# chanchanchan97/ICAFusion

Hardware: AMD Instinct MI355X
Metric: RGB/IR image-pairs/sec (two-stream forward + NMS) (higher is better)
Workload: dtype bf16

## Files before the change

icafusion_amd/_lib.py:

```python
import ctypes as C
import os

_HERE = os.path.dirname(os.path.abspath(__file__))
LIB_PATH = os.environ.get("ICAF_LIB") or os.path.join(_HERE, "lib", "libicaf.so")

F32, BF16, F16 = 0, 1, 2
ACT_NONE, ACT_SILU, ACT_GELU = 0, 1, 2


class ConvArgs(C.Structure):
    _fields_ = [
        ("x", C.c_void_p), ("w", C.c_void_p), ("bias", C.c_void_p), ("y", C.c_void_p), ("res", C.c_void_p),
        ("x_gs", C.c_longlong), ("w_gs", C.c_longlong), ("bias_gs", C.c_longlong), ("y_gs", C.c_longlong),
        ("res_gs", C.c_longlong),
        ("groups", C.c_int),
        ("B", C.c_int), ("H", C.c_int), ("W", C.c_int), ("Cin", C.c_int), ("ldx", C.c_int),
        ("Ho", C.c_int), ("Wo", C.c_int), ("Cout", C.c_int), ("ldy", C.c_int),
        ("kh", C.c_int), ("kw", C.c_int), ("sh", C.c_int), ("sw", C.c_int), ("ph", C.c_int), ("pw", C.c_int),
        ("ldr", C.c_int), ("Kp", C.c_int), ("act", C.c_int), ("dtype", C.c_int), ("out_dtype", C.c_int),
        ("alpha_acc", C.c_float * 2), ("alpha_res", C.c_float * 2),
        ("tile", C.c_int),
        ("pre", C.c_void_p), ("pre_h", C.c_int), ("pre_w", C.c_int), ("ldpre", C.c_int), ("pre_mode", C.c_int),
        ("w2", C.c_void_p), ("bias2", C.c_void_p), ("y2", C.c_void_p),
        ("w2_gs", C.c_longlong), ("bias2_gs", C.c_longlong), ("y2_gs", C.c_longlong),
# ... 2 lines not shown
        ("x2", C.c_void_p), ("x2_gs", C.c_longlong), ("ldx2", C.c_int), ("reserved2", C.c_int),
    ]


class BneckArgs(C.Structure):
    _fields_ = [("conv", ConvArgs), ("w1", C.c_void_p), ("bias1", C.c_void_p), ("w1_gs", C.c_longlong),
                ("bias1_gs", C.c_longlong), ("Kp1", C.c_int), ("shape", C.c_int),
                ("x2", C.c_void_p), ("x2_gs", C.c_longlong), ("ldx2", C.c_int), ("reserved", C.c_int)]


class Stem2Args(C.Structure):
    _fields_ = [("img", C.c_void_p), ("img_u8", C.c_int), ("ctot", C.c_int),
                ("dtype", C.c_int), ("nstreams", C.c_int), ("B", C.c_int), ("H", C.c_int), ("W", C.c_int),
                ("w0", C.c_void_p), ("bias0", C.c_void_p), ("w0_gs", C.c_longlong), ("bias0_gs", C.c_longlong),
                ("Kp0", C.c_int), ("C0", C.c_int),
                ("w1", C.c_void_p), ("bias1", C.c_void_p), ("w1_gs", C.c_longlong), ("bias1_gs", C.c_longlong),
                ("Kp1", C.c_int), ("C1", C.c_int),
                ("w2", C.c_void_p), ("bias2", C.c_void_p), ("w2_gs", C.c_longlong), ("bias2_gs", C.c_longlong),
                ("Kp2", C.c_int), ("C2", C.c_int),
                ("y", C.c_void_p), ("y_gs", C.c_longlong), ("ldy", C.c_int), ("reserved", C.c_int)]


class DmffArgs(C.Structure):
    _fields_ = [("x", C.c_void_p), ("qkv", C.c_void_p), ("y", C.c_void_p),
                ("wqkv", C.c_void_p), ("bqkv", C.c_void_p), ("wo", C.c_void_p), ("bo", C.c_void_p),
                ("w1", C.c_void_p), ("b1", C.c_void_p), ("w2", C.c_void_p), ("b2", C.c_void_p),
                ("ln_attn_gamma", C.c_void_p * 2), ("ln_attn_beta", C.c_void_p * 2),
                ("ln_mlp_gamma", C.c_void_p), ("ln_mlp_beta", C.c_void_p),
                ("wqkv_gs", C.c_longlong), ("bqkv_gs", C.c_longlong), ("wo_gs", C.c_longlong), ("bo_gs", C.c_longlong),
                ("w1_gs", C.c_longlong), ("b1_gs", C.c_longlong), ("w2_gs", C.c_longlong), ("b2_gs", C.c_longlong),
                ("x_gs", C.c_longlong), ("y_gs", C.c_longlong),
                ("dtype", C.c_int), ("B", C.c_int), ("N", C.c_int), ("C", C.c_int), ("heads", C.c_int), ("Kp", C.c_int),
                ("Kp4", C.c_int), ("hidden", C.c_int), ("ldy", C.c_int), ("reserved", C.c_int),
                ("eps_attn", C.c_float), ("eps_mlp", C.c_float),
                ("coef_res_attn", C.c_float * 2), ("coef_acc_attn", C.c_float * 2),
                ("coef_res_mlp", C.c_float * 2), ("coef_acc_mlp", C.c_float * 2), ("debug_clock", C.c_void_p),
                ("x32", C.c_void_p), ("y32", C.c_void_p)]


_p, _i, _ll, _f, _sz = C.c_void_p, C.c_int, C.c_longlong, C.c_float, C.c_size_t
SIGNATURES = {
    "icaf_last_error": (C.c_char_p, []),
    "icaf_set_option": (_i, [C.c_char_p, _i]),
    "icaf_version": (_i, []),
    "icaf_device_info": (_i, [C.POINTER(_i), C.POINTER(_i), C.c_char_p, _i]),
    "icaf_preprocess_nchw": (_i, [_p, _p, _i, _i, _i, _i, _i, _i, _i, _p]),
    "icaf_preprocess_u8": (_i, [_p, _p, _i, _i, _i, _i, _i, _i, _i, _i, _i, _i, _p]),
    "icaf_stem": (_i, [_p, _i, _i, _p, _p, _p, _i, _i, _i, _i, _i, _i, _i, _i, _ll, _ll, _ll, _p]),
    "icaf_stem2": (_i, [C.POINTER(Stem2Args), _p]),
    "icaf_conv2d": (_i, [C.POINTER(ConvArgs), _p]),
    "icaf_bottleneck": (_i, [C.POINTER(BneckArgs), _p]),
    "icaf_conv2d_kernel_name": (_i, [C.POINTER(ConvArgs), C.c_char_p, _i]),
    "icaf_conv2d_config_ids": (_i, [C.POINTER(_i), _i]),
    "icaf_sppf_pool": (_i, [_p, _i, _p, _p, _p, _i, _i, _i, _i, _i, _i, _i, _p]),
    "icaf_sppf_config": (_i, [_i, _i, _i, _i, C.POINTER(_i)]),
    "icaf_upsample_nearest": (_i, [_p, _i, _p, _i, _i, _i, _i, _i, _i, _i, _p]),
    "icaf_copy_channels": (_i, [_p, _i, _p, _i, _i, _ll, _i, _p]),
    "icaf_axpby": (_i, [_p, _i, _p, _i, _p, _i, _i, _ll, _i, _f, _f, _p]),
    "icaf_dmff_pool_tokens": (_i, [_p, _i, _p, _i, _p, _p, _p, _i, _i, _i, _i, _i, _i, _i, _i, _i, _i, _i,
                                   _f, _f, _f, _f, _p]),
    "icaf_layernorm": (_i, [_p, _p, _p, _p, _p, _p, _i, _ll, _i, _i, _f, _p]),
    "icaf_cross_attention": (_i, [_p, _p, _i, _i, _i, _i, _i, _p]),
    "icaf_cross_attention_config": (_i, [_i, _i, _i, _i, _i, C.POINTER(_i), C.POINTER(_i), C.POINTER(_i)]),
    "icaf_dmff_ln_qkv": (_i, [C.POINTER(DmffArgs), _p]),
    "icaf_dmff_attn_mlp": (_i, [C.POINTER(DmffArgs), _p]),
    "icaf_dmff_wide_ln_qkv": (_i, [C.POINTER(DmffArgs), _p]),
    "icaf_dmff_wide_proj_mlp": (_i, [C.POINTER(DmffArgs), _p, _p]),
    "icaf_dmff_wide_proj_mlp_split": (_i, [C.POINTER(DmffArgs), _p, _p, _i, _p]),
    "icaf_dmff_wide_reduce": (_i, [C.POINTER(DmffArgs), _p, _i, _p]),
    "icaf_dmff_attn_mlp_lds_bytes": (_i, [_i, _i, _i, _i, C.POINTER(_sz)]),
    "icaf_dmff_upsample_merge": (_i, [_p, _p, _i, _p, _i, _p, _i, _i, _i, _i, _i, _i, _i, _i, _p]),
    "icaf_detect_decode": (_i, [_p, _i, _p, _p, _p, _i, _i, _i, _i, _i, _ll, _ll, _f, C.POINTER(_f), _p]),
    "icaf_detect_decode_kernel": (_i, [_p, _i, _p, _p, _i, _i, _i, _i, _i, C.POINTER(_i)]),
    "icaf_detect_conv": (_i, [C.POINTER(ConvArgs), _p, _p, _p, _i, _i, _ll, _ll, _f, C.POINTER(_f), _p]),
    "icaf_match_predictions": (_i, [_p, _p, _i, _i, _p, _p, _i, _p, _p, _i, _p, _p, _p]),
    "icaf_nms_workspace_bytes": (_i, [_i, _ll, _i, _i, C.POINTER(_sz)]),
    "icaf_nms": (_i, [_p, _i, _ll, _i, _f, _f, _i, _i, C.POINTER(_i), _i, _i, _i, _f, _p, _p, _p, _p, _sz, _p]),
    "icaf_graph_begin": (_i, [_p]),
    "icaf_graph_end": (_i, [_p, C.POINTER(_p)]),
    "icaf_graph_launch": (_i, [_p, _p]),
    "icaf_graph_destroy": (_i, [_p]),
    "icaf_event_create": (_i, [C.POINTER(_p)]),
    "icaf_event_record": (_i, [_p, _p]),
    "icaf_stream_wait_event": (_i, [_p, _p]),
    "icaf_event_elapsed_ms": (_i, [_p, _p, C.POINTER(_f)]),
    "icaf_event_destroy": (_i, [_p]),
    "icaf_stream_sync": (_i, [_p]),
}

_LIB = None


class IcafError(RuntimeError):
    pass


def lib():
    global _LIB
    if _LIB is None:
        if not os.path.exists(LIB_PATH):
            raise IcafError(f"{LIB_PATH} not found — build it with `python -m icafusion_amd.build` "
                            "(hipcc --offload-arch=gfx950); icafusion_amd has no CPU / PyTorch fallback")
        import torch
        handle = C.CDLL(LIB_PATH)
        for name, (res, args) in SIGNATURES.items():
            try:
# ... 17 lines not shown
```

icafusion_amd/csrc/conv_common.h:

```cpp
#pragma once
#include "icaf_common.h"

namespace icaf {

struct ConvP {
    const void* x; const void* w; const float* bias; void* y; const void* res;
    long long x_gs, w_gs, bias_gs, y_gs, res_gs;
    int B, H, W, Cin, ldx, Ho, Wo, Cout, ldy, kh, kw, sh, sw, ph, pw, ldr, Kp, act;
    int M, K, nchunks, mtiles, ntiles;
    int vec_y, vec_r;
    unsigned int x_bytes, w_bytes;
    float alpha_acc[2], alpha_res[2];
    const float* pre; int pre_h, pre_w, ldpre, pre_mode;
    const void* w1; const float* bias1;
    long long w1_gs, bias1_gs; int Kp1; unsigned int w1_bytes;
    const void* w2; const float* bias2; void* y2;
    long long w2_gs, bias2_gs, y2_gs; int Kp2, Cout2, ldy2, vec_y2, keep1; unsigned int w2_bytes;
    const void* x2; long long x2_gs; int ldx2;
};

constexpr int ROWB = 64;
constexpr int ROWS = 80;
constexpr int NTHREADS = 256;

int ctile_conv_check(const icaf_conv_args* a, const ConvP& p, int shape);
int launch_ctile(const icaf_conv_args* a, const ConvP& p, int shape, hipStream_t s);
const char* ctile_tag(int shape);
int stream_check(const icaf_conv_args* a, const ConvP& p, int shape);
int launch_stream(const icaf_conv_args* a, const ConvP& p, int shape, hipStream_t s);
const char* stream_tag(int shape);
int wreg_check(const icaf_conv_args* a, const ConvP& p, int shape);
int launch_wreg(const icaf_conv_args* a, const ConvP& p, int shape, hipStream_t s);
const char* wreg_tag(int shape);
int cstream_check(const icaf_conv_args* a, const ConvP& p, int shape);
int launch_cstream(const icaf_conv_args* a, const ConvP& p, int shape, hipStream_t s);
const char* cstream_tag(int shape);
int cwide_check(const icaf_conv_args* a, const ConvP& p, int shape);
int launch_cwide(const icaf_conv_args* a, const ConvP& p, int shape, hipStream_t s);
const char* cwide_tag(int shape);
int launch_bneck(const icaf_conv_args* a, const ConvP& p, int shape, hipStream_t s);

template <int ACT, int DT = ICAF_F32> __device__ __forceinline__ float apply_act(float v) {
    if constexpr (ACT == ICAF_ACT_SILU) return silu_f(v);
    else if constexpr (ACT == ICAF_ACT_GELU) return DT == ICAF_F32 ? gelu_f(v) : gelu_fast_f(v);
    else return v;
}
template <int ACT, int DT = ICAF_F32> __device__ __forceinline__ void apply_act4(const float (&x)[4], float (&y)[4]) {
    if constexpr (ACT == ICAF_ACT_SILU) silu4_f(x, y);
    else {
#pragma unroll
        for (int j = 0; j < 4; ++j) y[j] = apply_act<ACT, DT>(x[j]);
    }
}

__device__ __forceinline__ int xcd_tile(int ntile_total) {
    const int bid = blockIdx.x, q = ntile_total >> 3, r = ntile_total & 7, xcd = bid & 7, idx = bid >> 3;
    return (xcd < r ? xcd * (q + 1) : r * (q + 1) + (xcd - r) * q) + idx;
}

#ifndef ICAF_EPI_FAST
#define ICAF_EPI_FAST 1
#endif
// ... 400 lines not shown
```

icafusion_amd/csrc/detect.hip:

```cpp
#pragma clang fp contract(off)
#include "icaf_common.h"
#include "stream_core.h"
#include <cstdlib>

namespace icaf {

struct Anchors { float v[16]; };
int conv_prepare(const icaf_conv_args* a, ConvP& p);

struct DetectDiv { FastDiv no, nx, ny, na; };

template <bool I32>
__global__ __launch_bounds__(256) void detect_decode_kernel(const float* __restrict__ p, int ldp, float* __restrict__ z,
                                                            float* __restrict__ logits, float* __restrict__ raw, int B, int ny, int nx,
                                                            int na, int no, long long rows_total, long long row_offset, float stride,
                                                            Anchors anc, DetectDiv dv) {
    const long long total = (long long)B * na * ny * nx * no;
    for (long long e = (long long)blockIdx.x * blockDim.x + threadIdx.x; e < total; e += (long long)gridDim.x * blockDim.x) {
        int o, x, y, a, b;
        if constexpr (I32) {
            unsigned int q, r;
            fd_divmod((unsigned int)e, dv.no, q, r);
            o = (int)r;
            fd_divmod(q, dv.nx, q, r);
// ... 107 lines not shown
            const int nl = col0 + 8 * qd + 4 * hi;
#pragma unroll
            for (int b = 0; b < TM; ++b) {
                const int ml = row0 + b * 32 + l31;
                f32x4 v;
#pragma unroll
                for (int j = 0; j < 4; ++j) v[j] = acc[b][4 * qd + j] + bq[qd][j];
                *(f32x4*)(stg + ml * SO + nl * 4) = v;
            }
        }
    }
    __device__ __forceinline__ void flush(const unsigned char* stg, int m0, int n0, int tid) const {
        if (tid >= 128 * NA) return;
        const int row = tid / NA, a = tid - row * NA;
        const unsigned int pix = (unsigned int)(m0 + row);
        if ((int)pix >= M) return;
        unsigned int t, x, b, y;
        fd_divmod(pix, dnx, t, x);
        fd_divmod(t, dny, b, y);
        const float* src = (const float*)(stg + row * SO) + a * NO;
        float v[NO];
#pragma unroll
        for (int k = 0; k < NO; k += 2) { const float2 q2 = *(const float2*)(src + k); v[k] = q2.x; v[k + 1] = q2.y; }
        const long long cell = ((long long)a * ny + y) * nx + x;
        const long long zrow = (long long)b * rows_total + row_offset + cell;
        float o[NO];
#pragma unroll
        for (int k = 0; k < NO; ++k) {
            const float sg = 1.0f / (1.0f + expf(-v[k]));
            float out = sg;
            if (k == 0) out = ((sg * 2.0f - 0.5f) + (float)x) * stride;
            else if (k == 1) out = ((sg * 2.0f - 0.5f) + (float)y) * stride;
            else if (k == 2 || k == 3) {
                const float d = sg * 2.0f;
                out = (d * d) * anc.v[2 * a + (k - 2)];
            }
            o[k] = out;
        }
        float* zr = z + zrow * NO;
#pragma unroll
        for (int k = 0; k < NO; k += 2) *(float2*)(zr + k) = float2{o[k], o[k + 1]};
        if (raw) {
            float* rr = raw + (((long long)b * NA) * ny * nx + cell) * NO;
#pragma unroll
            for (int k = 0; k < NO; k += 2) *(float2*)(rr + k) = float2{v[k], v[k + 1]};
        }
        if (logits) {
#pragma unroll
            for (int k = 5; k < NO; ++k) logits[zrow * (NO - 5) + (k - 5)] = v[k];
        }
    }
};

template <int DT, int NA, int NO>
__global__ __launch_bounds__(512) void detect_conv_kernel(const ConvP p, const DetectEpi<NA, NO> epi) {
    stream_gemm<DT, 64, 1>(p, epi);
}

template <int DT, int NA, int NO>
static int launch_detect_conv(const ConvP& p, const DetectEpi<NA, NO>& epi, hipStream_t s) {
    constexpr int LDS = 3 * (128 + 64) * 128 + 128 * DetectEpi<NA, NO>::SO;
    ConvP q = p;
    q.mtiles = (p.M + 127) / 128;
    q.ntiles = 1;
    q.nchunks = p.K / 64;
    int dev = 0, cus = 256;
    ICAF_HIP(hipGetDevice(&dev));
    ICAF_HIP(hipDeviceGetAttribute(&cus, hipDeviceAttributeMultiprocessorCount, dev));
    const int grid = cus & ~7;
    ICAF_LDS_OPTIN((detect_conv_kernel<DT, NA, NO>), LDS);
    detect_conv_kernel<DT, NA, NO><<<dim3((unsigned)grid, 1, 1), dim3(512), LDS, s>>>(q, epi);
    ICAF_LAUNCH_CHECK();
    return ICAF_OK;
}

}

using namespace icaf;

enum { DETECT_PIXEL = 0, DETECT_ELEMENT = 1 };

static int detect_select(const float* p, int ldp, const float* z, const float* raw, int B, int ny, int nx, int na, int no) {
    const bool aligned = ldp % 2 == 0 && ((uintptr_t)p & 7) == 0 && ((uintptr_t)z & 7) == 0 && (!raw || ((uintptr_t)raw & 7) == 0);
    const bool pixel = na == 3 && (no == 6 || no == 8 || no == 14) && aligned && (long long)B * ny * nx < (1ll << 31) && !g_opt.detect_elementwise;
    return pixel ? DETECT_PIXEL : DETECT_ELEMENT;
}

extern "C" int icaf_detect_decode_kernel(const float* p, int ldp, const float* z, const float* raw, int B, int ny, int nx, int na, int no,
                                         int* kernel) {
    if (!p || !z || !kernel) return fail(ICAF_ERR_ARG, "icaf_detect_decode_kernel: null pointer");
    if (na < 1 || na > 8 || no < 6 || ldp < na * no) return fail(ICAF_ERR_ARG, "icaf_detect_decode_kernel: bad na/no/ldp");
    if (B < 1 || ny < 1 || nx < 1) return fail(ICAF_ERR_ARG, "icaf_detect_decode_kernel: empty level");
    *kernel = detect_select(p, ldp, z, raw, B, ny, nx, na, no);
    return ICAF_OK;
}

extern "C" int icaf_detect_decode(const float* p, int ldp, float* z, float* logits, float* raw, int B, int ny, int nx, int na, int no,
                                  long long rows_total, long long row_offset, float stride, const float* anchors_px, icaf_stream_t s) {
    if (!p || !z || !anchors_px) return fail(ICAF_ERR_ARG, "icaf_detect_decode: null pointer");
    if (na < 1 || na > 8 || no < 6 || ldp < na * no) return fail(ICAF_ERR_ARG, "icaf_detect_decode: bad na/no/ldp");
    if (row_offset + (long long)na * ny * nx > rows_total) return fail(ICAF_ERR_ARG, "icaf_detect_decode: level does not fit in z");
    Anchors anc;
    for (int i = 0; i < 16; ++i) anc.v[i] = i < 2 * na ? anchors_px[i] : 0.0f;
    const long long cells = (long long)B * na * ny * nx * no;
    long long blocks = (cells + 255) / 256;
    if (blocks > 256 * 32) blocks = 256 * 32;
    if (B < 1 || ny < 1 || nx < 1) return fail(ICAF_ERR_ARG, "icaf_detect_decode: empty level");
    if (detect_select(p, ldp, z, raw, B, ny, nx, na, no) == DETECT_PIXEL) {
        if (no == 6) return launch_detect_pixel<3, 6>(p, ldp, z, logits, raw, B, ny, nx, rows_total, row_offset, stride, anc, S(s));
        if (no == 8) return launch_detect_pixel<3, 8>(p, ldp, z, logits, raw, B, ny, nx, rows_total, row_offset, stride, anc, S(s));
        if (no == 14) return launch_detect_pixel<3, 14>(p, ldp, z, logits, raw, B, ny, nx, rows_total, row_offset, stride, anc, S(s));
    }
    const DetectDiv dv{make_fastdiv((unsigned)no), make_fastdiv((unsigned)nx), make_fastdiv((unsigned)ny), make_fastdiv((unsigned)na)};
    if (cells < (1ll << 31))
        hipLaunchKernelGGL(detect_decode_kernel<true>, dim3((unsigned)blocks), dim3(256), 0, S(s), p, ldp, z, logits, raw, B, ny, nx, na,
                           no, rows_total, row_offset, stride, anc, dv);
    else
        hipLaunchKernelGGL(detect_decode_kernel<false>, dim3((unsigned)blocks), dim3(256), 0, S(s), p, ldp, z, logits, raw, B, ny, nx, na,
                           no, rows_total, row_offset, stride, anc, dv);
    ICAF_LAUNCH_CHECK();
    return ICAF_OK;
}

extern "C" int icaf_detect_conv(const icaf_conv_args* a, float* z, float* logits, float* raw, int na, int no, long long rows_total,
// ... 27 lines not shown
```

icafusion_amd/csrc/igemm_stream.hip:

```cpp
#include "stream_core.h"

namespace icaf {

template <int DT, int BN, int ACT, bool PRE = false>
struct StoreEpi {
    using E = Elem<DT>;
    static constexpr int SO = BN * E::BYTES + 16;
    typename E::type* yg; float alpha_acc; int M, Cout, ldy;
    const typename E::type* rg; float alpha_res; int ldr;
    const float* pre; int pre_h, pre_w, ldpre, pre_mode, Ho, Wo;
    template <int TM>
    __device__ __forceinline__ void stage(const f32x16 (&acc)[TM], const f32x4 (&bq)[4], unsigned char* stg, int row0, int col0, int l31, int hi, int m0, int n0) const {
        const float* pt[PRE ? TM : 1][4];
        float plx[PRE ? TM : 1], ply[PRE ? TM : 1];
        if constexpr (PRE) {
#pragma clang fp contract(off)
            const float sy = (float)pre_h / (float)Ho, sx = (float)pre_w / (float)Wo;
#pragma unroll
            for (int b = 0; b < TM; ++b) {
                const int m = m0 + row0 + b * 32 + l31;
                const int mm = m < M ? m : 0;
                const int wo = mm % Wo, t = mm / Wo, ho = t % Ho, bi = t / Ho;
                float fy = ((float)ho + 0.5f) * sy - 0.5f, fx = ((float)wo + 0.5f) * sx - 0.5f;
                fy = fy < 0.0f ? 0.0f : fy;
// ... 24 lines not shown
                const int ml = row0 + b * 32 + l31;
                float pv[4] = {0.f, 0.f, 0.f, 0.f};
                if constexpr (PRE) if (n0 + nl < Cout) {
                    const f32x4 t00 = *(const f32x4*)(pt[b][0] + n0 + nl), t01 = *(const f32x4*)(pt[b][1] + n0 + nl);
                    const f32x4 t10 = *(const f32x4*)(pt[b][2] + n0 + nl), t11 = *(const f32x4*)(pt[b][3] + n0 + nl);
                    {
#pragma clang fp contract(off)
                        const float wx0 = 1.0f - plx[b], wy0 = 1.0f - ply[b];
#pragma unroll
                        for (int j = 0; j < 4; ++j) {
                            const float top = t00[j] * wx0 + t01[j] * plx[b];
                            const float bot = t10[j] * wx0 + t11[j] * plx[b];
                            pv[j] = top * wy0 + bot * ply[b];
                        }
                    }
                }
                float v[4];
#pragma unroll
                for (int j = 0; j < 4; ++j) v[j] = acc[b][4 * qd + j] + bq[qd][j] + pv[j];
                apply_act4<ACT, DT>(v, v);
#pragma unroll
                for (int j = 0; j < 4; ++j) v[j] *= alpha_acc;
                u32x2 pk;
                if constexpr (DT == ICAF_BF16) { pk[0] = pack2_bf16(v[0], v[1]); pk[1] = pack2_bf16(v[2], v[3]); }
                else { pk[0] = pack2_f16(v[0], v[1]); pk[1] = pack2_f16(v[2], v[3]); }
                *(u32x2*)(stg + ml * SO + nl * E::BYTES) = pk;
            }
        }
    }
    __device__ __forceinline__ void flush(const unsigned char* stg, int m0, int n0, int tid) const {
        constexpr int VPR = BN / E::VEC;
        constexpr int NIT = 128 * VPR / 512;
#pragma unroll
        for (int itv = 0; itv < NIT; ++itv) {
            const int idx = tid + itv * 512;
            const int row = idx / VPR, cv = idx - row * VPR;
            const int m = m0 + row, n = n0 + cv * E::VEC;
            u32x4 sv = *(const u32x4*)(stg + row * SO + cv * 16);
            if (m < M && n < Cout) {
                if (rg) {
                    float v[E::VEC], r[E::VEC];
                    unpack16<DT>(sv, v);
                    unpack16<DT>(*(const u32x4*)(rg + (long long)m * ldr + n), r);
#pragma unroll
                    for (int j = 0; j < E::VEC; ++j) v[j] = __builtin_fmaf(alpha_res, r[j], v[j]);
                    sv = pack16<DT>(v);
                }
                *(u32x4*)(yg + (long long)m * ldy + n) = sv;
            }
        }
    }
};

template <int DT, int BN, int ACT, int MODE, bool PRE = false>
__global__ __launch_bounds__(512) void igemm_stream_kernel(const ConvP p) {
    using E = Elem<DT>;
    const int g = blockIdx.z;
    const StoreEpi<DT, BN, ACT, PRE> epi{(typename E::type*)p.y + g * p.y_gs, p.alpha_acc[g], p.M, p.Cout, p.ldy,
                                         p.res ? (const typename E::type*)p.res + g * p.res_gs : nullptr, p.alpha_res[g], p.ldr,
                                         p.pre, p.pre_h, p.pre_w, p.ldpre, p.pre_mode, p.Ho, p.Wo};
    stream_gemm<DT, BN, MODE>(p, epi);
}

const char* stream_tag(int shape) { return shape == 1 ? "128x128" : shape == 2 ? "128x64" : "?"; }

static int stream_grid(int groups, int* wgx) {
    int dev = 0, cus = 256;
    ICAF_HIP(hipGetDevice(&dev));
    ICAF_HIP(hipDeviceGetAttribute(&cus, hipDeviceAttributeMultiprocessorCount, dev));
    *wgx = ((cus / (groups > 0 ? groups : 1)) & ~7) >> 3;
    return ICAF_OK;
}

int stream_check(const icaf_conv_args* a, const ConvP& p, int shape) {
    if (shape < 1 || shape > 2) return fail(ICAF_ERR_ARG, "igemm_stream: unknown shape %d", shape);
    if (a->dtype == ICAF_F32 || a->out_dtype != a->dtype) return fail(ICAF_ERR_UNSUPPORTED, "igemm_stream: 16-bit types, out dtype == dtype");
    if ((a->Cin * 2) % 128) return fail(ICAF_ERR_UNSUPPORTED, "igemm_stream: Cin * 2 bytes must be a multiple of 128 (Cin = %d)", a->Cin);
    if (a->w2) return fail(ICAF_ERR_UNSUPPORTED, "igemm_stream: no chained layer");
    if (a->pre && (a->act != ICAF_ACT_SILU || a->kh != 1 || a->kw != 1 || a->sh != 1 || a->sw != 1 || a->ph || a->pw || a->groups != 1))
        return fail(ICAF_ERR_UNSUPPORTED, "igemm_stream: the pre-activation term is built for 1x1 SiLU layers (one group)");
    if (a->res && !p.vec_r) return fail(ICAF_ERR_UNSUPPORTED, "igemm_stream: the residual must take 16-byte vectors");
    if (p.x_bytes == 0) return fail(ICAF_ERR_UNSUPPORTED, "igemm_stream: operand exceeds the 2 GiB buffer-descriptor range");
    if (!p.vec_y || a->Cout % 8) return fail(ICAF_ERR_UNSUPPORTED, "igemm_stream: y must take 16-byte vectors (ldy %% 8, Cout %% 8, alignment)");
    if (shape == 1 && a->Cout <= 64) return fail(ICAF_ERR_UNSUPPORTED, "igemm_stream 128x128: Cout = %d <= 64 (use 128x64)", a->Cout);
    int wgx = 0;
    const int st = stream_grid(a->groups, &wgx);
    if (st) return st;
    const int ntiles = (p.Cout + (shape == 1 ? 128 : 64) - 1) / (shape == 1 ? 128 : 64);
    if (wgx < ntiles || wgx % ntiles) return fail(ICAF_ERR_UNSUPPORTED, "igemm_stream: %d channel tiles do not divide the %d workgroups of an XCD", ntiles, wgx);
    return ICAF_OK;
}

template <int DT, int BN, int ACT>
static int launch_stream_cfg(const ConvP& p, int groups, hipStream_t s) {
    constexpr int LDS = 3 * (128 + BN) * 128 + 128 * (BN * 2 + 16);
    ConvP q = p;
    q.mtiles = (p.M + 127) / 128;
    q.ntiles = (p.Cout + BN - 1) / BN;
    q.nchunks = p.K / 64;
    int dev = 0, wgx = 0;
    ICAF_HIP(hipGetDevice(&dev));
    if (dev < 0 || dev >= ICAF_MAX_DEVICES) return fail(ICAF_ERR_UNSUPPORTED, "device ordinal %d", dev);
    int st = stream_grid(groups, &wgx);
    if (st) return st;
    const int grid = wgx << 3;
    if (wgx < q.ntiles || wgx % q.ntiles) return fail(ICAF_ERR_UNSUPPORTED, "igemm_stream: %d channel tiles do not divide the %d workgroups of an XCD", q.ntiles, wgx);
    const bool plain = q.kh == 1 && q.kw == 1 && q.sh == 1 && q.sw == 1 && q.ph == 0 && q.pw == 0;
    auto go = [&](auto kern) -> int {
        ICAF_LDS_OPTIN(kern, LDS);
        kern<<<dim3((unsigned)grid, 1, (unsigned)groups), dim3(512), LDS, s>>>(q);
        ICAF_LAUNCH_CHECK();
        return ICAF_OK;
    };
    if constexpr (ACT == ICAF_ACT_SILU) { if (p.pre) return go(igemm_stream_kernel<DT, BN, ACT, 1, true>); }
    if (plain) return go(igemm_stream_kernel<DT, BN, ACT, 1>);
    return go(igemm_stream_kernel<DT, BN, ACT, 2>);
}

template <int DT, int BN>
static int launch_stream_act(const ConvP& p, int groups, hipStream_t s) {
    if (p.act == ICAF_ACT_SILU) return launch_stream_cfg<DT, BN, ICAF_ACT_SILU>(p, groups, s);
    if (p.act == ICAF_ACT_GELU) return launch_stream_cfg<DT, BN, ICAF_ACT_GELU>(p, groups, s);
    return launch_stream_cfg<DT, BN, ICAF_ACT_NONE>(p, groups, s);
}

int launch_stream(const icaf_conv_args* a, const ConvP& p, int shape, hipStream_t s) {
    if (a->dtype == ICAF_BF16) return shape == 1 ? launch_stream_act<ICAF_BF16, 128>(p, a->groups, s) : launch_stream_act<ICAF_BF16, 64>(p, a->groups, s);
    return shape == 1 ? launch_stream_act<ICAF_F16, 128>(p, a->groups, s) : launch_stream_act<ICAF_F16, 64>(p, a->groups, s);
}

}
```

icafusion_amd/csrc/stream_core.h:

```cpp
#pragma once
#include "conv_common.h"

namespace icaf {

template <int DT, int BN, int MODE, class EPI>
__device__ __forceinline__ void stream_gemm(const ConvP& p, const EPI& epi) {
    using E = Elem<DT>;
    static_assert(DT != ICAF_F32, "16-bit types");
    constexpr int BM = 128, RB = 128, NS = 3, NW = 8;
    constexpr int WN = 32, WM = BN == 128 ? 64 : 32;
    constexpr int TM = WM / 32, TN = 1;
    constexpr int WAVES_M = BM / WM;
    constexpr int VEC = E::VEC;
    constexpr int RPI = 8;
    constexpr int NA = BM / RPI / NW, NB = BN / RPI / NW;
    constexpr int PER = NA + NB;
    constexpr int STAGE = (BM + BN) * RB;
    constexpr int NSTEP = RB / 32;
    constexpr int RING = NS * STAGE;
    static_assert(NA >= 1 && NB >= 1 && (BN == 128 || BN == 64), "tile shape");
    extern __shared__ __attribute__((aligned(1024))) unsigned char lds[];
    unsigned char* stg = lds + RING;

    const int tid = threadIdx.x, lane = tid & 63, l31 = lane & 31, hi = lane >> 5;
    const int wave = __builtin_amdgcn_readfirstlane(tid >> 6);
    const int g = blockIdx.z;
    const int wm = wave % WAVES_M, wn = wave / WAVES_M;

    const __amdgpu_buffer_rsrc_t xr = __builtin_amdgcn_make_buffer_rsrc(
        (void*)((const typename E::type*)p.x + g * p.x_gs), 0, p.x_bytes, 0x00020000);
    const __amdgpu_buffer_rsrc_t wr = __builtin_amdgcn_make_buffer_rsrc(
        (void*)((const typename E::type*)p.w + g * p.w_gs), 0, p.w_bytes, 0x00020000);
    constexpr unsigned OOB = 0x80000000u;

    const int rsub = lane >> 3;
    const int dkey = ((wave & 1) << 2) | (rsub >> 1);
    const int lslot = (lane & 7) ^ dkey;

    const int xcd = blockIdx.x & 7, lb = blockIdx.x >> 3, wgx = gridDim.x >> 3;
    const int per_xcd = (p.mtiles + 7) >> 3, m_lo = xcd * per_xcd, m_hi = min(m_lo + per_xcd, p.mtiles);
    const int nt = lb % p.ntiles, mstride = wgx / p.ntiles, m_first = m_lo + lb / p.ntiles;
    const int n0 = nt * BN;
    const int nch = p.nchunks;

    int it = m_first, ic = 0;
    int kc = 0, ky = 0, kx = 0;
    unsigned ia_off[NA], iw_off[NB];
    int ia_h0[NA], ia_w0[NA];
#pragma unroll
    for (int i = 0; i < NB; ++i)
        iw_off[i] = ((unsigned)(n0 + (wave + NW * i) * RPI + rsub) * (unsigned)p.Kp + (unsigned)(lslot * VEC)) * E::BYTES;
    auto issue_setup = [&]() {
        const bool live = it < m_hi;
#pragma unroll
        for (int i = 0; i < NA; ++i) {
            const int m = it * BM + (wave + NW * i) * RPI + rsub;
            const bool ok = live && m < p.M;
            if constexpr (MODE == 1) {
                ia_off[i] = ok ? ((unsigned)m * (unsigned)p.ldx + (unsigned)(lslot * VEC)) * E::BYTES : OOB;
            } else {
                const int mm = ok ? m : 0;
                const int wo = mm % p.Wo, t = mm / p.Wo, ho = t % p.Ho, b = t / p.Ho;
                ia_h0[i] = ok ? ho * p.sh - p.ph : -0x10000;
                ia_w0[i] = wo * p.sw - p.pw;
                ia_off[i] = (unsigned)b * (unsigned)(p.H * p.W) * (unsigned)p.ldx * (unsigned)E::BYTES
                          + (unsigned)((ia_h0[i] * p.W + ia_w0[i]) * p.ldx + lslot * VEC) * E::BYTES;
            }
        }
    };
    auto issue_part = [&](int stage, int part) {
        unsigned char* st = lds + stage * STAGE;
        const unsigned koff = (unsigned)ic * RB;
        unsigned tap_delta = 0;
        if constexpr (MODE == 2) tap_delta = (unsigned)((ky * p.W + kx) * p.ldx + kc) * E::BYTES;
#pragma unroll
        for (int i = 0; i < NA; ++i) {
            if (i % NSTEP != part) continue;
            unsigned voff;
            if constexpr (MODE == 1) {
                voff = ia_off[i] == OOB ? OOB : ia_off[i] + koff;
            } else {
                const int h = ia_h0[i] + ky, w = ia_w0[i] + kx;
                const bool ok = (unsigned)h < (unsigned)p.H && (unsigned)w < (unsigned)p.W;
                voff = ok ? ia_off[i] + tap_delta : OOB;
            }
            __builtin_amdgcn_raw_ptr_buffer_load_lds(xr, (lds_ptr_t)(st + (wave + NW * i) * 1024), 16, voff, 0, 0, 0);
        }
#pragma unroll
        for (int i = 0; i < NB; ++i) {
            if ((NA + i) % NSTEP != part) continue;
            const unsigned voff = it < m_hi ? iw_off[i] + koff : OOB;
            __builtin_amdgcn_raw_ptr_buffer_load_lds(wr, (lds_ptr_t)(st + BM * RB + (wave + NW * i) * 1024), 16, voff, 0, 0, 0);
        }
    };
    auto issue_advance = [&]() {
        if constexpr (MODE == 2) {
            kc += RB / E::BYTES;
            if (kc >= p.Cin) { kc = 0; if (++kx == p.kw) { kx = 0; ++ky; } }
        }
        if (++ic == nch) {
            ic = 0; kc = 0; ky = 0; kx = 0;
            it += mstride;
            issue_setup();
        }
    };

    const float* __restrict__ bias = p.bias ? p.bias + g * p.bias_gs : nullptr;
    f32x4 bq[4];
#pragma unroll
    for (int qd = 0; qd < 4; ++qd) {
        const int n = n0 + wn * WN + 8 * qd + 4 * hi;
        const bool okn = bias && n < p.Cout;
        const float* bp = okn ? bias + n : (const float*)p.w;
        const f32x4 t = *(const f32x4*)bp;
        bq[qd] = okn ? t : f32x4{0.f, 0.f, 0.f, 0.f};
    }
#pragma unroll
    for (int qd = 0; qd < 4; ++qd) asm volatile("" : "+v"(bq[qd]));

    if (m_first >= m_hi) return;

    const int fkey = (l31 >> 1) & 7;
    int foff[NSTEP];
#pragma unroll
    for (int s = 0; s < NSTEP; ++s) foff[s] = l31 * RB + (((2 * s + hi) ^ fkey) << 4);

    issue_setup();
#pragma unroll
    for (int s = 0; s < NS; ++s) {
#pragma unroll
        for (int part = 0; part < NSTEP; ++part) issue_part(s, part);
        issue_advance();
    }

    int q = 0;
    for (int mt = m_first; mt < m_hi; mt += mstride) {
        const int m0 = mt * BM;
        f32x16 acc[TM];
#pragma unroll
        for (int b = 0; b < TM; ++b)
#pragma unroll
            for (int r = 0; r < 16; ++r) acc[b][r] = 0.0f;
        for (int c = 0; c < nch; ++c, ++q) {
            wait_vmcnt<PER>();
            asm volatile("s_waitcnt lgkmcnt(0)" ::: "memory");
            __builtin_amdgcn_s_barrier();
            const int sq = q % NS;
            const unsigned char* a_s = lds + sq * STAGE;
            const unsigned char* b_s = a_s + BM * RB;
            u32x4 fp[NSTEP][TM], fw[NSTEP];
#pragma unroll
            for (int s = 0; s < NSTEP; ++s) {
#pragma unroll
                for (int b = 0; b < TM; ++b) fp[s][b] = *(const u32x4*)(a_s + (wm * WM + b * 32) * RB + foff[s]);
                fw[s] = *(const u32x4*)(b_s + (wn * WN) * RB + foff[s]);
            }
            const int sfree = (q + NS - 1) % NS;
#pragma unroll
            for (int s = 0; s < NSTEP; ++s) {
#pragma unroll
                for (int b = 0; b < TM; ++b) mma_step<DT>(acc[b], fw[s], fp[s][b]);
                if (q > 0) issue_part(sfree, s);
            }
            if (q > 0) issue_advance();
        }

        epi.stage(acc, bq, stg, wm * WM, wn * WN, l31, hi, m0, n0);
        lds_barrier();
        epi.flush(stg, m0, n0, tid);
    }
    wait_vmcnt<0>();
}


}
```

include/icaf.h:

```cpp
#ifndef ICAF_H
#define ICAF_H

#include <stddef.h>

#ifdef __cplusplus
extern "C" {
#endif

typedef void* icaf_stream_t;

enum { ICAF_F32 = 0, ICAF_BF16 = 1, ICAF_F16 = 2 };
enum { ICAF_ACT_NONE = 0, ICAF_ACT_SILU = 1, ICAF_ACT_GELU = 2 };
enum { ICAF_OK = 0, ICAF_ERR_ARG = -1, ICAF_ERR_HIP = -2, ICAF_ERR_UNSUPPORTED = -3 };

const char* icaf_last_error(void);
int icaf_set_option(const char* name, int value);
int icaf_version(void);
int icaf_device_info(int* cu_count, int* lds_bytes, char* arch, int arch_len);

int icaf_preprocess_nchw(const float* img, void* out, int dtype, int B, int C, int H, int W, int Cpad, int mode,
                         icaf_stream_t s);
int icaf_preprocess_u8(const unsigned char* img, void* out, int dtype, int B, int Ctot, int c0, int C, int nstreams,
                       int H, int W, int Cpad, int mode, icaf_stream_t s);

// ... 12 lines not shown
int icaf_stem2(const icaf_stem2_args* a, icaf_stream_t s);

typedef struct icaf_conv_args {
    const void* x;
    const void* w;
    const float* bias;
    void* y;
    const void* res;
    long long x_gs, w_gs, bias_gs, y_gs, res_gs;
    int groups;
    int B, H, W, Cin, ldx;
    int Ho, Wo, Cout, ldy;
    int kh, kw, sh, sw, ph, pw;
    int ldr;
    int Kp;
    int act;
    int dtype;
    int out_dtype;
    float alpha_acc[2];
    float alpha_res[2];
    int tile;
    const float* pre;
    int pre_h, pre_w, ldpre;
    int pre_mode;
    const void* w2;
    const float* bias2;
    void* y2;
    long long w2_gs, bias2_gs, y2_gs;
    int Kp2, Cout2, ldy2;
    int chain_keep;
    const void* wf;
    long long wf_gs;
    const void* x2;
    long long x2_gs;
    int ldx2, reserved2;
} icaf_conv_args;

int icaf_conv2d(const icaf_conv_args* a, icaf_stream_t s);

typedef struct icaf_bneck_args {
    icaf_conv_args conv;
    const void* w1;
    const float* bias1;
    long long w1_gs, bias1_gs;
    int Kp1;
    int shape;
    const void* x2;
    long long x2_gs;
    int ldx2, reserved;
} icaf_bneck_args;
int icaf_bottleneck(const icaf_bneck_args* a, icaf_stream_t s);
int icaf_conv2d_kernel_name(const icaf_conv_args* a, char* buf, int buf_len);
int icaf_conv2d_config_ids(int* ids, int cap);

int icaf_sppf_pool(const void* x, int ldx, void* y1, void* y2, void* y3, int ldy, int dtype, int B, int H, int W,
                   int C, int k, icaf_stream_t s);
int icaf_sppf_config(int dtype, int H, int W, int C, int* vpb);
int icaf_upsample_nearest(const void* x, int ldx, void* y, int ldy, int dtype, int B, int H, int W, int C,
                          int scale, icaf_stream_t s);
int icaf_copy_channels(const void* x, int ldx, void* y, int ldy, int dtype, long long rows, int C,
                       icaf_stream_t s);
int icaf_axpby(const void* x0, int ld0, const void* x1, int ld1, void* y, int ldy, int dtype, long long rows, int C,
               float a, float b, icaf_stream_t s);

int icaf_dmff_pool_tokens(const void* fea_rgb, int ld_rgb, const void* fea_ir, int ld_ir, const float* pos_rgb,
                          const float* pos_ir, void* tokens, int dtype, int B, int H, int W, int C, int th, int tw,
                          int kh, int kw, int sh, int sw, float w1_rgb, float w2_rgb, float w1_ir, float w2_ir,
                          icaf_stream_t s);
int icaf_layernorm(const void* x, void* y, const float* gamma0, const float* beta0, const float* gamma1,
                   const float* beta1, int dtype, long long rows_per_group, int C, int groups, float eps,
                   icaf_stream_t s);
int icaf_cross_attention(const void* qkv, void* out, int dtype, int B, int N, int C, int heads, icaf_stream_t s);
int icaf_cross_attention_config(int dtype, int B, int N, int C, int heads, int* dkp, int* qsplit, int* remap);
int icaf_dmff_upsample_merge(const void* tokens, const void* fea_rgb, int ld_rgb, const void* fea_ir, int ld_ir,
                             void* out, int ldo, int dtype, int B, int H, int W, int C, int th, int tw,
                             icaf_stream_t s);

int icaf_detect_decode(const float* p, int ldp, float* z, float* logits, float* raw, int B, int ny, int nx, int na,
                       int no, long long rows_total, long long row_offset, float stride, const float* anchors_px,
                       icaf_stream_t s);
int icaf_detect_decode_kernel(const float* p, int ldp, const float* z, const float* raw, int B, int ny, int nx, int na,
                              int no, int* kernel);
int icaf_detect_conv(const icaf_conv_args* a, float* z, float* logits, float* raw, int na, int no, long long rows_total,
                     long long row_offset, float stride, const float* anchors_px, icaf_stream_t s);

typedef struct icaf_dmff_args {
    const void* x; void* qkv; void* y;
    const void* wqkv; const float* bqkv;
    const void* wo; const float* bo;
    const void* w1; const float* b1;
    const void* w2; const float* b2;
    const float* ln_attn_gamma[2]; const float* ln_attn_beta[2];
    const float* ln_mlp_gamma; const float* ln_mlp_beta;
    long long wqkv_gs, bqkv_gs, wo_gs, bo_gs, w1_gs, b1_gs, w2_gs, b2_gs, x_gs, y_gs;
    int dtype, B, N, C, heads, Kp, Kp4, hidden, ldy, reserved;
    float eps_attn, eps_mlp;
    float coef_res_attn[2], coef_acc_attn[2], coef_res_mlp[2], coef_acc_mlp[2];
    void* debug_clock;
    const float* x32; float* y32;
} icaf_dmff_args;
int icaf_dmff_ln_qkv(const icaf_dmff_args* a, icaf_stream_t s);
int icaf_dmff_attn_mlp(const icaf_dmff_args* a, icaf_stream_t s);
int icaf_dmff_wide_ln_qkv(const icaf_dmff_args* a, icaf_stream_t s);
int icaf_dmff_wide_proj_mlp(const icaf_dmff_args* a, const void* att, icaf_stream_t s);
int icaf_dmff_wide_proj_mlp_split(const icaf_dmff_args* a, const void* att, float* partial, int ksplit, icaf_stream_t s);
int icaf_dmff_wide_reduce(const icaf_dmff_args* a, const float* partial, int ksplit, icaf_stream_t s);
// ... 26 lines not shown
```

Measured before the change: 17200.

## Keep weight panel resident in LDS for 1x1 stream GEMM with deeper activation ring

For plain 1x1 stream-GEMM layers, including the detect head, whose full weight slice fits within an LDS budget, the weights are loaded once per workgroup into LDS. The activation ring then uses the remaining space for a deeper pipeline of up to five stages. This removes repeated weight streaming per M tile and allows more loads in flight, with vmcnt waits adjusted to the depth. The cost is higher LDS use, which may reduce occupancy, plus a larger up-front weight load that only pays off when a workgroup processes several tiles.

```diff
diff --git a/icafusion_amd/_lib.py b/icafusion_amd/_lib.py
--- a/icafusion_amd/_lib.py
+++ b/icafusion_amd/_lib.py
@@ -78,6 +78,7 @@
     "icaf_bottleneck": (_i, [C.POINTER(BneckArgs), _p]),
     "icaf_conv2d_kernel_name": (_i, [C.POINTER(ConvArgs), C.c_char_p, _i]),
     "icaf_conv2d_config_ids": (_i, [C.POINTER(_i), _i]),
+    "icaf_stream_lds_plan": (_i, [_i, _i, _i, _i, _i, C.POINTER(_i), C.POINTER(_i), C.POINTER(_i)]),
     "icaf_sppf_pool": (_i, [_p, _i, _p, _p, _p, _i, _i, _i, _i, _i, _i, _i, _p]),
     "icaf_sppf_config": (_i, [_i, _i, _i, _i, C.POINTER(_i)]),
     "icaf_upsample_nearest": (_i, [_p, _i, _p, _i, _i, _i, _i, _i, _i, _i, _p]),
diff --git a/icafusion_amd/csrc/conv_common.h b/icafusion_amd/csrc/conv_common.h
--- a/icafusion_amd/csrc/conv_common.h
+++ b/icafusion_amd/csrc/conv_common.h
@@ -8,6 +8,7 @@
     long long x_gs, w_gs, bias_gs, y_gs, res_gs;
     int B, H, W, Cin, ldx, Ho, Wo, Cout, ldy, kh, kw, sh, sw, ph, pw, ldr, Kp, act;
     int M, K, nchunks, mtiles, ntiles;
+    int stream_depth;
     int vec_y, vec_r;
     unsigned int x_bytes, w_bytes;
     float alpha_acc[2], alpha_res[2];
diff --git a/icafusion_amd/csrc/detect.hip b/icafusion_amd/csrc/detect.hip
--- a/icafusion_amd/csrc/detect.hip
+++ b/icafusion_amd/csrc/detect.hip
@@ -183,14 +183,13 @@
     }
 };
 
-template <int DT, int NA, int NO>
+template <int DT, int NA, int NO, bool RES = false>
 __global__ __launch_bounds__(512) void detect_conv_kernel(const ConvP p, const DetectEpi<NA, NO> epi) {
-    stream_gemm<DT, 64, 1>(p, epi);
+    stream_gemm<DT, 64, 1, RES>(p, epi);
 }
 
 template <int DT, int NA, int NO>
 static int launch_detect_conv(const ConvP& p, const DetectEpi<NA, NO>& epi, hipStream_t s) {
-    constexpr int LDS = 3 * (128 + 64) * 128 + 128 * DetectEpi<NA, NO>::SO;
     ConvP q = p;
     q.mtiles = (p.M + 127) / 128;
     q.ntiles = 1;
@@ -199,8 +198,15 @@
     ICAF_HIP(hipGetDevice(&dev));
     ICAF_HIP(hipDeviceGetAttribute(&cus, hipDeviceAttributeMultiprocessorCount, dev));
     const int grid = cus & ~7;
-    ICAF_LDS_OPTIN((detect_conv_kernel<DT, NA, NO>), LDS);
-    detect_conv_kernel<DT, NA, NO><<<dim3((unsigned)grid, 1, 1), dim3(512), LDS, s>>>(q, epi);
+    const StreamLds lp = stream_lds_plan(64, q.K, DetectEpi<NA, NO>::SO, true, stream_max_tiles(q.mtiles, 1, grid >> 3));
+    q.stream_depth = lp.depth;
+    if (lp.resident) {
+        ICAF_LDS_OPTIN((detect_conv_kernel<DT, NA, NO, true>), lp.bytes);
+        detect_conv_kernel<DT, NA, NO, true><<<dim3((unsigned)grid, 1, 1), dim3(512), lp.bytes, s>>>(q, epi);
+    } else {
+        ICAF_LDS_OPTIN((detect_conv_kernel<DT, NA, NO>), lp.bytes);
+        detect_conv_kernel<DT, NA, NO><<<dim3((unsigned)grid, 1, 1), dim3(512), lp.bytes, s>>>(q, epi);
+    }
     ICAF_LAUNCH_CHECK();
     return ICAF_OK;
 }
diff --git a/icafusion_amd/csrc/igemm_stream.hip b/icafusion_amd/csrc/igemm_stream.hip
--- a/icafusion_amd/csrc/igemm_stream.hip
+++ b/icafusion_amd/csrc/igemm_stream.hip
@@ -100,14 +100,14 @@
     }
 };
 
-template <int DT, int BN, int ACT, int MODE, bool PRE = false>
+template <int DT, int BN, int ACT, int MODE, bool PRE = false, bool RES = false>
 __global__ __launch_bounds__(512) void igemm_stream_kernel(const ConvP p) {
     using E = Elem<DT>;
     const int g = blockIdx.z;
     const StoreEpi<DT, BN, ACT, PRE> epi{(typename E::type*)p.y + g * p.y_gs, p.alpha_acc[g], p.M, p.Cout, p.ldy,
                                          p.res ? (const typename E::type*)p.res + g * p.res_gs : nullptr, p.alpha_res[g], p.ldr,
                                          p.pre, p.pre_h, p.pre_w, p.ldpre, p.pre_mode, p.Ho, p.Wo};
-    stream_gemm<DT, BN, MODE>(p, epi);
+    stream_gemm<DT, BN, MODE, RES>(p, epi);
 }
 
 const char* stream_tag(int shape) { return shape == 1 ? "128x128" : shape == 2 ? "128x64" : "?"; }
@@ -141,7 +141,6 @@
 
 template <int DT, int BN, int ACT>
 static int launch_stream_cfg(const ConvP& p, int groups, hipStream_t s) {
-    constexpr int LDS = 3 * (128 + BN) * 128 + 128 * (BN * 2 + 16);
     ConvP q = p;
     q.mtiles = (p.M + 127) / 128;
     q.ntiles = (p.Cout + BN - 1) / BN;
@@ -154,14 +153,18 @@
     const int grid = wgx << 3;
     if (wgx < q.ntiles || wgx % q.ntiles) return fail(ICAF_ERR_UNSUPPORTED, "igemm_stream: %d channel tiles do not divide the %d workgroups of an XCD", q.ntiles, wgx);
     const bool plain = q.kh == 1 && q.kw == 1 && q.sh == 1 && q.sw == 1 && q.ph == 0 && q.pw == 0;
+    const StreamLds lp = stream_lds_plan(BN, q.K, StoreEpi<DT, BN, ACT>::SO, plain, stream_max_tiles(q.mtiles, q.ntiles, wgx));
+    q.stream_depth = lp.depth;
     auto go = [&](auto kern) -> int {
-        ICAF_LDS_OPTIN(kern, LDS);
-        kern<<<dim3((unsigned)grid, 1, (unsigned)groups), dim3(512), LDS, s>>>(q);
+        ICAF_LDS_OPTIN(kern, lp.bytes);
+        kern<<<dim3((unsigned)grid, 1, (unsigned)groups), dim3(512), lp.bytes, s>>>(q);
         ICAF_LAUNCH_CHECK();
         return ICAF_OK;
     };
-    if constexpr (ACT == ICAF_ACT_SILU) { if (p.pre) return go(igemm_stream_kernel<DT, BN, ACT, 1, true>); }
-    if (plain) return go(igemm_stream_kernel<DT, BN, ACT, 1>);
+    if constexpr (ACT == ICAF_ACT_SILU) {
+        if (p.pre) return lp.resident ? go(igemm_stream_kernel<DT, BN, ACT, 1, true, true>) : go(igemm_stream_kernel<DT, BN, ACT, 1, true>);
+    }
+    if (plain) return lp.resident ? go(igemm_stream_kernel<DT, BN, ACT, 1, false, true>) : go(igemm_stream_kernel<DT, BN, ACT, 1>);
     return go(igemm_stream_kernel<DT, BN, ACT, 2>);
 }
 
@@ -178,3 +181,11 @@
 }
 
 }
+
+extern "C" int icaf_stream_lds_plan(int bn, int K, int staging_stride, int plain, int max_tiles, int* resident, int* depth, int* bytes) {
+    if ((bn != 128 && bn != 64) || K < 64 || K % 64 || staging_stride < 16 || !resident || !depth || !bytes)
+        return icaf::fail(ICAF_ERR_ARG, "icaf_stream_lds_plan: bad arguments");
+    const icaf::StreamLds lp = icaf::stream_lds_plan(bn, K, staging_stride, plain != 0, max_tiles);
+    *resident = lp.resident; *depth = lp.depth; *bytes = lp.bytes;
+    return ICAF_OK;
+}
diff --git a/icafusion_amd/csrc/stream_core.h b/icafusion_amd/csrc/stream_core.h
--- a/icafusion_amd/csrc/stream_core.h
+++ b/icafusion_amd/csrc/stream_core.h
@@ -1,12 +1,34 @@
 #pragma once
 #include "conv_common.h"
 
+#ifndef ICAF_STREAM_LDS_BUDGET
+#define ICAF_STREAM_LDS_BUDGET (160 * 1024)
+#endif
+
 namespace icaf {
 
-template <int DT, int BN, int MODE, class EPI>
+struct StreamLds { int resident, depth, w_bytes, stage_bytes, bytes; };
+constexpr int STREAM_DMAX = 5;
+constexpr StreamLds stream_lds_plan(int bn, int K, int so, bool plain, int max_tiles) {
+    const int stg = 128 * so, w = (K / 64) * bn * 128;
+    const int room = ICAF_STREAM_LDS_BUDGET - stg - w;
+    const int fit = room > 0 ? room / (128 * 128) : 0;
+    if (plain && max_tiles >= 2 && w <= 64 * 1024 && fit >= 3) {
+        const int d = fit < STREAM_DMAX ? fit : STREAM_DMAX;
+        return StreamLds{1, d, w, 128 * 128, w + d * 128 * 128 + stg};
+    }
+    return StreamLds{0, 3, 0, (128 + bn) * 128, 3 * (128 + bn) * 128 + stg};
+}
+constexpr int stream_max_tiles(int mtiles, int ntiles, int wgx) {
+    const int per_xcd = (mtiles + 7) >> 3, slots = wgx / ntiles;
+    return slots > 0 ? (per_xcd + slots - 1) / slots : 0;
+}
+
+template <int DT, int BN, int MODE, bool RES, class EPI>
 __device__ __forceinline__ void stream_gemm(const ConvP& p, const EPI& epi) {
     using E = Elem<DT>;
     static_assert(DT != ICAF_F32, "16-bit types");
+    static_assert(!RES || MODE == 1, "the resident form is built for 1x1 layers");
     constexpr int BM = 128, RB = 128, NS = 3, NW = 8;
     constexpr int WN = 32, WM = BN == 128 ? 64 : 32;
     constexpr int TM = WM / 32, TN = 1;
@@ -14,13 +36,16 @@
     constexpr int VEC = E::VEC;
     constexpr int RPI = 8;
     constexpr int NA = BM / RPI / NW, NB = BN / RPI / NW;
-    constexpr int PER = NA + NB;
-    constexpr int STAGE = (BM + BN) * RB;
+    constexpr int PER = RES ? NA : NA + NB;
+    constexpr int STAGE = (RES ? BM : BM + BN) * RB;
     constexpr int NSTEP = RB / 32;
-    constexpr int RING = NS * STAGE;
     static_assert(NA >= 1 && NB >= 1 && (BN == 128 || BN == 64), "tile shape");
+    static_assert((STREAM_DMAX - 2) * NA <= 18, "vmcnt immediate");
     extern __shared__ __attribute__((aligned(1024))) unsigned char lds[];
-    unsigned char* stg = lds + RING;
+    const int nch = p.nchunks;
+    const int D = RES ? p.stream_depth : NS;
+    unsigned char* ring = lds + (RES ? nch * BN * RB : 0);
+    unsigned char* stg = ring + D * STAGE;
 
     const int tid = threadIdx.x, lane = tid & 63, l31 = lane & 31, hi = lane >> 5;
     const int wave = __builtin_amdgcn_readfirstlane(tid >> 6);
@@ -41,7 +66,6 @@
     const int per_xcd = (p.mtiles + 7) >> 3, m_lo = xcd * per_xcd, m_hi = min(m_lo + per_xcd, p.mtiles);
     const int nt = lb % p.ntiles, mstride = wgx / p.ntiles, m_first = m_lo + lb / p.ntiles;
     const int n0 = nt * BN;
-    const int nch = p.nchunks;
 
     int it = m_first, ic = 0;
     int kc = 0, ky = 0, kx = 0;
@@ -69,7 +93,7 @@
         }
     };
     auto issue_part = [&](int stage, int part) {
-        unsigned char* st = lds + stage * STAGE;
+        unsigned char* st = ring + stage * STAGE;
         const unsigned koff = (unsigned)ic * RB;
         unsigned tap_delta = 0;
         if constexpr (MODE == 2) tap_delta = (unsigned)((ky * p.W + kx) * p.ldx + kc) * E::BYTES;
@@ -86,11 +110,13 @@
             }
             __builtin_amdgcn_raw_ptr_buffer_load_lds(xr, (lds_ptr_t)(st + (wave + NW * i) * 1024), 16, voff, 0, 0, 0);
         }
-#pragma unroll
-        for (int i = 0; i < NB; ++i) {
-            if ((NA + i) % NSTEP != part) continue;
-            const unsigned voff = it < m_hi ? iw_off[i] + koff : OOB;
-            __builtin_amdgcn_raw_ptr_buffer_load_lds(wr, (lds_ptr_t)(st + BM * RB + (wave + NW * i) * 1024), 16, voff, 0, 0, 0);
+        if constexpr (!RES) {
+#pragma unroll
+            for (int i = 0; i < NB; ++i) {
+                if ((NA + i) % NSTEP != part) continue;
+                const unsigned voff = it < m_hi ? iw_off[i] + koff : OOB;
+                __builtin_amdgcn_raw_ptr_buffer_load_lds(wr, (lds_ptr_t)(st + BM * RB + (wave + NW * i) * 1024), 16, voff, 0, 0, 0);
+            }
         }
     };
     auto issue_advance = [&]() {
@@ -125,15 +151,22 @@
 #pragma unroll
     for (int s = 0; s < NSTEP; ++s) foff[s] = l31 * RB + (((2 * s + hi) ^ fkey) << 4);
 
+    if constexpr (RES) {
+        for (int c = 0; c < nch; ++c)
+#pragma unroll
+            for (int i = 0; i < NB; ++i)
+                __builtin_amdgcn_raw_ptr_buffer_load_lds(wr, (lds_ptr_t)(lds + c * BN * RB + (wave + NW * i) * 1024), 16,
+                                                         iw_off[i] + (unsigned)c * RB, 0, 0, 0);
+    }
     issue_setup();
-#pragma unroll
-    for (int s = 0; s < NS; ++s) {
+    for (int s = 0; s < D; ++s) {
 #pragma unroll
         for (int part = 0; part < NSTEP; ++part) issue_part(s, part);
         issue_advance();
     }
 
     int q = 0;
+    int sq = 0, sfree = D - 1;
     for (int mt = m_first; mt < m_hi; mt += mstride) {
         const int m0 = mt * BM;
         f32x16 acc[TM];
@@ -142,12 +175,14 @@
 #pragma unroll
             for (int r = 0; r < 16; ++r) acc[b][r] = 0.0f;
         for (int c = 0; c < nch; ++c, ++q) {
-            wait_vmcnt<PER>();
+            if constexpr (!RES) wait_vmcnt<(NS - 2) * PER>();
+            else if (D >= 5) wait_vmcnt<3 * PER>();
+            else if (D == 4) wait_vmcnt<2 * PER>();
+            else wait_vmcnt<PER>();
             asm volatile("s_waitcnt lgkmcnt(0)" ::: "memory");
             __builtin_amdgcn_s_barrier();
-            const int sq = q % NS;
-            const unsigned char* a_s = lds + sq * STAGE;
-            const unsigned char* b_s = a_s + BM * RB;
+            const unsigned char* a_s = ring + sq * STAGE;
+            const unsigned char* b_s = RES ? lds + c * BN * RB : a_s + BM * RB;
             u32x4 fp[NSTEP][TM], fw[NSTEP];
 #pragma unroll
             for (int s = 0; s < NSTEP; ++s) {
@@ -155,7 +190,6 @@
                 for (int b = 0; b < TM; ++b) fp[s][b] = *(const u32x4*)(a_s + (wm * WM + b * 32) * RB + foff[s]);
                 fw[s] = *(const u32x4*)(b_s + (wn * WN) * RB + foff[s]);
             }
-            const int sfree = (q + NS - 1) % NS;
 #pragma unroll
             for (int s = 0; s < NSTEP; ++s) {
 #pragma unroll
@@ -163,6 +197,8 @@
                 if (q > 0) issue_part(sfree, s);
             }
             if (q > 0) issue_advance();
+            sfree = sq;
+            sq = sq + 1 == D ? 0 : sq + 1;
         }
 
         epi.stage(acc, bq, stg, wm * WM, wn * WN, l31, hi, m0, n0);
diff --git a/include/icaf.h b/include/icaf.h
--- a/include/icaf.h
+++ b/include/icaf.h
@@ -88,6 +88,7 @@
 int icaf_bottleneck(const icaf_bneck_args* a, icaf_stream_t s);
 int icaf_conv2d_kernel_name(const icaf_conv_args* a, char* buf, int buf_len);
 int icaf_conv2d_config_ids(int* ids, int cap);
+int icaf_stream_lds_plan(int bn, int K, int staging_stride, int plain, int max_tiles, int* resident, int* depth, int* bytes);
 
 int icaf_sppf_pool(const void* x, int ldx, void* y1, void* y2, void* y3, int ldy, int dtype, int B, int H, int W,
                    int C, int k, icaf_stream_t s);
```

New measurement: 17150. No clear change (-0.3%).
